# ducha-aiki/pydegensac

Measured on AMD Instinct MI355X. Metric: models/sec, findFundamentalMatrix @2000 corrs (LO-RANSAC + DEGENSAC, batched pairs), higher is better.
Workload: dtype f64

## Files before the change

pydegensac_amd/csrc/dg_f_lo.h:

```cpp
#ifndef DG_F_LO_H
#define DG_F_LO_H

__device__ __forceinline__ unsigned dg_hash_list(const int *list, int count, bool small_ids = false)
{
    if (count <= 0) return 0;
    const int lane = (int)(threadIdx.x & 63);
    unsigned hash = (unsigned)__builtin_amdgcn_readfirstlane(count * 4), tmp;
#define DG_HSTEP(v_) { unsigned v = (unsigned)(v_); \
        hash += v & 0xffffu; tmp = ((v >> 16) << 11) ^ hash; hash = (hash << 16) ^ tmp; hash += hash >> 11; }
#define DG_HSTEP16(v_) { unsigned v = (unsigned)(v_); \
        hash += v; hash = (hash << 16) ^ hash; hash += hash >> 11; }
    int k = 0;
    int cur = (lane < count) ? list[lane] : 0;
    int n1 = (64 + lane < count) ? list[64 + lane] : 0, n2 = (128 + lane < count) ? list[128 + lane] : 0, n3 = (192 + lane < count) ? list[192 + lane] : 0;
    for (; k + 64 <= count; k += 64) {
        const int n4 = (k + 256 + lane < count) ? list[k + 256 + lane] : 0;
        if (small_ids) {
#pragma unroll
            for (int i = 0; i < 64; i++) DG_HSTEP16(__builtin_amdgcn_readlane(cur, i))
        } else {
#pragma unroll
            for (int i = 0; i < 64; i++) DG_HSTEP(__builtin_amdgcn_readlane(cur, i))
        }
        cur = n1; n1 = n2; n2 = n3; n3 = n4;
// ... 64 lines not shown
        DG_LT(4);
        if (wv == 1) {
            unsigned hash = dg_hash_list(inliers, (int)Sc.I, n < 65536);
            if ((tid & 63) == 0) {
                int ret = dg_ht_contains(c.ht, hash, (int)Sc.I, iterID);
                if (ret == -1) dg_ht_insert(c.ht, hash, (int)Sc.I, iterID);
                S->itmp[0] = (ret != -1 && ret != iterID) ? 1 : 0;
            }
        } else if (wv == 0 && fit) {
            const int cnt = (int)r2.nL; int use = cnt, id;
            if (tid == 0) S->rng_save = S->rng;
            DG_WSYNC();
            if (8 < cnt) { dg_randsubset_wave(&S->rng, alt, cnt, 8, tid, &id); use = 8; }
            else id = tid < cnt ? alt[tid] : 0;
            if (tid < use) {
                dg_pt q = dg_ldpt<LDSPTS>(c.P, id);
                double *px = S->lsq.px + 4*tid; px[0] = q.x1; px[1] = q.y1; px[2] = q.x2; px[3] = q.y2;
                if (mk_ex == DG_K_FDS) S->lsq.part[0][tid] = dg_exFDs_w(fl, q.x1, q.y1, q.x2, q.y2);
                else { double w; dg_exFDsSym(fl, q.x1, q.y1, q.x2, q.y2, &w); S->lsq.part[0][tid] = w; }
            }
            DG_WSYNC();
            dg_u2f_small_w(&S->lsq, S->lsq.px, S->lsq.part[0], use, S->ftmp, tid);
        }
        __syncthreads();
        DG_LT(5);
        if (S->itmp[0]) {
            if (fit && tid == 0) S->rng = S->rng_save;
            __syncthreads();
            DG_TRACE(c, 13, 0, 0); return zero;
        }
        if (improve) {
            maxS = Sc; *kind0 = mk_ex;
            if (tid < 9) f[tid] = fl[tid];
        }
        DG_TRACE(c, 14, r2.nL, 0);
        for (int j = tid; j < (int)r2.nL; j += DG_T) inliers[j] = alt[j];
        if (tid < 9 && fit) fl[tid] = S->ftmp[tid];
        __syncthreads();
        DG_LT(6);
        if (!fit) return maxS;
        ths -= dth;
    }
    dg_pass_cfg c3 = dg_cfg0(n); c3.wantJ = 1; c3.thJ = th; c3.list = inliers; c3.thL = th;
    DG_LT(0);
    dg_pass_res r3 = dg_f_pass(c, fl, mk_full, c3); c.n_fds++;
    dg_dump_resid(c, rrow + 4, fl, mk_full);
    DG_LT(7);
    DG_TRACE(c, 12, r3.I, r3.J);
    if (maxS.J < r3.J) {
        maxS = zero; maxS.I = r3.I; maxS.J = r3.J; *kind0 = mk_full;
        __syncthreads();
        if (tid < 9) f[tid] = fl[tid];
        __syncthreads();
    }
    return maxS;
}

template <int LDSPTS>
__device__ __noinline__ dg_score dg_inFrani_serial(CTX &c, int ninl, double th, double *Fout, int *iterID,
                                               int mk_full, int mk_ex, int *kindBest)
{
    dg_f_shared *S = c.S; const int tid = c.tid;
    int *inliers = c.K->L[0], *intbuff = c.K->L[1], *intbuff_best = c.K->L[2];
    dg_score maxS = {0, 0, 0, 0};
    *kindBest = mk_full;
    if (ninl < 16) {
        if (c.rrun) { for (size_t j = tid; j < (size_t)(DG_RESIDS_M - 2) * c.n; j += DG_T) c.rrun[2 * (size_t)c.n + j] = 0.; __syncthreads(); }
        return maxS;
    }
    int ssiz = ninl / 2; if (ssiz > 14) ssiz = 14;
    const int wave = tid >> 6, lane = tid & 63;
    if (tid == 0) S->n_ahead = 0;
    for (int i = 0; i < DG_RAN_REP; i++) {
        DG_LT(0);
        __syncthreads();
        int taken = 0;
        if (S->n_ahead > 0) {
            if (tid < 64) {
                int hit = -1;
                for (int k = 0; k < S->n_ahead; k++) {
                    const int *a = (const int *)&S->rng, *b = (const int *)&S->ahead[k].before;
                    const bool same = lane < 31 ? a[lane] == b[lane] : (lane == 31 ? S->rng.f == S->ahead[k].before.f : (lane == 32
                        ? S->rng.b == S->ahead[k].before.b : true));
                    if (hit < 0 && __ballot(!same) == 0ull) hit = k;
                }
                if (hit >= 0) {
                    const dg_lo_ahead *h = &S->ahead[hit];
                    if (lane < 2 * ssiz && h->pos[lane] >= 0) inliers[h->pos[lane]] = h->val[lane];
                    if (lane < 9) S->f[lane] = h->F[lane];
                    DG_WSYNC();
                    if (lane == 0) S->rng = h->after;
                }
                if (lane == 0) S->itmp[29] = hit;
            }
            __syncthreads();
            taken = S->itmp[29] >= 0;
        }
        if (!taken) {
            if (tid < 64) { int id; dg_randsubset_wave(&S->rng, inliers, ninl, ssiz, tid, &id); dg_gather_wave(c, id, ssiz, S->lsq.px, tid); }
            __syncthreads();
            if (wave == 0) {
                dg_u2f_small_w(&S->lsq, S->lsq.px, 0, ssiz, S->f, tid);
            } else if (DG_AHEAD_ON && wave <= DG_LO_AHEAD && ssiz > 8 && i + 1 < DG_RAN_REP) {
                const int sub = wave == 1 ? 2 : wave == 2 ? 3 : wave == 3 ? 4 : wave == 4 ? 1 : 5;
                dg_lo_ahead *h = &S->ahead[wave - 1];
                dg_wave_ws *w = &S->ww[wave];
                if (lane == 0) { h->before = S->rng; for (int q = 0; q < 8 * sub; q++) dg_rand(&h->before); h->after = h->before; }
                DG_WSYNC();
                int id;
                dg_randsubset_wave_ahead(&h->after, inliers, ninl, ssiz, lane, &id, h->pos, h->val);
                dg_gather_wave(c, id, ssiz, w->px, lane);
                DG_WSYNC();
                dg_u2f_norm_w(w, w->px, (const double *)0, ssiz, h->F, lane);
            }
            if (tid == 0) S->n_ahead = (DG_AHEAD_ON && ssiz > 8 && i + 1 < DG_RAN_REP) ? DG_LO_AHEAD : 0;
        } else if (tid == 0) S->n_ahead = 0;
        DG_LT(8);
#ifdef DG_LO_PROF
        if (c.tid == 0) { if (taken) c.S->lt[10]++; else c.S->lt[11]++; }
#endif
        __syncthreads();
        int k0;
        ++*iterID;
        dg_dump_resid(c, 2 + 6 * i, S->f, mk_full);
        dg_score Sc = dg_iterF(c, intbuff, th, DG_TC * th, S->f, *iterID, mk_full, mk_ex, &k0, 2 + 6 * i + 1);
        if (maxS.J < Sc.J) {
            maxS = Sc; *kindBest = k0;
            __syncthreads();
            if (tid < 9) Fout[tid] = S->f[tid];
            for (int j = tid; j < (int)maxS.I; j += DG_T) intbuff_best[j] = intbuff[j];
            __syncthreads();
        }
    }
    __syncthreads();
    for (int j = tid; j < (int)maxS.I; j += DG_T) inliers[j] = intbuff_best[j];
    __syncthreads();
    return maxS;
}

template <int LDSPTS>
__device__ __forceinline__ dg_pass_res dg_f_wpass(const dg_pt *P, int n, int kind, const double *Fm , double thJ, int *la_, double thL, int *lb_,
    double thL2,
                                               double *tile, int lane)
{
    n = __builtin_amdgcn_readfirstlane(n); kind = __builtin_amdgcn_readfirstlane(kind);
    double F[9];
#pragma unroll
    for (int i = 0; i < 9; i++) F[i] = Fm[i];
    return dg_wpass_impl<LDSPTS>(P, n, [&](const dg_pt &q) { return dg_Ferr(kind, F, q); }, thJ, la_, thL, lb_, thL2, tile, lane);
}

#define DG_LO_ASSUMED_DRAWS 16
template <int LDSPTS>
__device__ __forceinline__ void dg_lo_rep_wave(CTX &c, dg_lo_log *lg, int ssiz, double th, int mk_full, int mk_ex, int lane, int wave)
{
    ssiz = __builtin_amdgcn_readfirstlane(ssiz); wave = __builtin_amdgcn_readfirstlane(wave);
    dg_f_shared *S = c.S; const int n = c.n, nm = c.K->n_max; const dg_pt *P = c.P;
    dg_wave_ws *w = &S->ww[wave];
    int *ib = c.K->wlist + (size_t)wave * nm;
    int *alt = (int *)(c.K->wstage + (size_t)wave * nm);
    double *jb = w->Z;
    double *f = w->F, *fl = w->H, *wts = w->cpx, *ftmp = w->cpx + 8;
    const bool small_ids = n < 65536;
#ifdef DG_LO_PROF
    long long tw_ = wall_clock64(); const long long tw0_ = tw_;
#define DG_RW(i) do { if (wave == 0 && lane == 0) { long long t_ = wall_clock64(); S->lt[i] += t_ - tw_; tw_ = t_; } } while (0)
#else
#define DG_RW(i) do {} while (0)
#endif
    auto stale = [&]() {
        int bad = 0;
        if (lane < wave) { const int d = __hip_atomic_load(&S->lo[lane].pub, __ATOMIC_RELAXED, __HIP_MEMORY_SCOPE_WORKGROUP);
            bad = d >= 0 && d != DG_LO_ASSUMED_DRAWS; }
        return __ballot(bad) != 0ull;
    };
    int drawn = 0;
    DG_WSYNC();
    dg_gather_wave(c, lane < ssiz ? lg->ids[lane] : 0, ssiz, w->px, lane);
    DG_WSYNC();
    dg_u2f_small_wave(w, w->px, (const double *)0, ssiz, f, lane);
    DG_RW(8);
    const dg_pass_res r0 = dg_f_wpass<LDSPTS>(P, n, mk_full, f, th, ib, th * DG_MWM, (int *)0, 0.0, jb, lane);
    DG_RW(9);
    unsigned mI = r0.I; double mJ = r0.J; int kind0 = mk_full;
    if (lane == 0) { lg->I0 = (int)r0.I; lg->drew0 = 0; lg->nit = 0; lg->has_fin = 0; }
    if (mI < 8) { if (lane == 0) { lg->I = 0; lg->J = 0; lg->kind0 = mk_full; __hip_atomic_store(&lg->pub, 0, __ATOMIC_RELAXED, __HIP_MEMORY_SCOPE_WORKGROUP);
        } DG_WSYNC(); return; }
    {
        const int cnt = (int)r0.nL; int id;
        if (8 < cnt) { dg_randsubset_wave(&lg->g, ib, cnt, 8, lane, &id); if (lane == 0) lg->drew0 = 8; drawn += 8; }
        else id = lane < cnt ? ib[lane] : 0;
        const int use = 8 < cnt ? 8 : cnt;
        DG_WSYNC();
        dg_gather_wave(c, id, use, w->px, lane);
        DG_WSYNC();
        dg_u2f_small_wave(w, w->px, (const double *)0, use, fl, lane);
    }
    DG_RW(10);
    double ths = DG_TC * th; const double dth = (ths - th) / DG_ILSQ_ITERS;
    int it = 0, ended = 0;
    for (; it < DG_ILSQ_ITERS; it++) {
        if (stale()) { if (lane == 0) lg->aborted = 1; DG_WSYNC(); return; }
        const dg_pass_res r1 = dg_f_wpass<LDSPTS>(P, n, mk_ex, fl, th, ib, th, alt, ths * DG_MWM, jb, lane);
        const int improve = __builtin_amdgcn_readfirstlane(mJ < r1.J);
        unsigned nL2 = r1.nL2;
        if (improve) { const dg_pass_res r2 = dg_f_wpass<LDSPTS>(P, n, kind0, f, 0.0, alt, ths * DG_MWM, (int *)0, 0.0, jb, lane); nL2 = r2.nL; }
        const int fit = __builtin_amdgcn_readfirstlane(nL2 >= 8);
        DG_WSYNC();
        DG_RW(9);
        const unsigned hash = dg_hash_list(ib, (int)r1.I, small_ids);
        if (lane == 0) { lg->it[it].hash = hash; lg->it[it].I = (int)r1.I; lg->it[it].drew = 0; lg->nit = it + 1; }
        { const bool known = dg_ht_known_wave(c.ht, hash, (int)r1.I, lane); DG_RW(11);
            if (known) { ended = 2; break; } }
        if (fit) {
            const int cnt = (int)nL2; int id;
            if (8 < cnt) {
                dg_randsubset_wave(&lg->g, alt, cnt, 8, lane, &id); if (lane == 0) lg->it[it].drew = 8; drawn += 8;
                if (drawn > DG_LO_ASSUMED_DRAWS && lane == 0) __hip_atomic_store(&lg->pub, drawn, __ATOMIC_RELAXED, __HIP_MEMORY_SCOPE_WORKGROUP);
            }
            else id = lane < cnt ? alt[lane] : 0;
            const int use = 8 < cnt ? 8 : cnt;
            DG_WSYNC();
            if (lane < use) {
                const dg_pt q = dg_ldpt<LDSPTS>(P, id);
                double *px = w->px + 4 * lane; px[0] = q.x1; px[1] = q.y1; px[2] = q.x2; px[3] = q.y2;
                if (mk_ex == DG_K_FDS) wts[lane] = dg_exFDs_w(fl, q.x1, q.y1, q.x2, q.y2);
                else { double ww_; dg_exFDsSym(fl, q.x1, q.y1, q.x2, q.y2, &ww_); wts[lane] = ww_; }
            }
            DG_WSYNC();
            dg_u2f_small_wave(w, w->px, wts, use, ftmp, lane);
        }
        if (improve) { mI = r1.I; mJ = r1.J; kind0 = mk_ex; DG_WSYNC(); if (lane < 9) f[lane] = fl[lane]; DG_WSYNC(); }
        for (int j = lane; j < (int)nL2; j += 64) ib[j] = alt[j];
        DG_WSYNC();
        if (lane < 9 && fit) fl[lane] = ftmp[lane];
        DG_WSYNC();
        DG_RW(10);
        if (!fit) { ended = 1; break; }
        ths -= dth;
    }
    if (!ended) {
        const dg_pass_res r3 = dg_f_wpass<LDSPTS>(P, n, mk_full, fl, th, ib, th, (int *)0, 0.0, jb, lane);
        if (lane == 0) lg->has_fin = 1;
        if (__builtin_amdgcn_readfirstlane(mJ < r3.J)) { mI = r3.I; mJ = r3.J; kind0 = mk_full; DG_WSYNC(); if (lane < 9) f[lane] = fl[lane]; DG_WSYNC(); }
    }
    DG_WSYNC();
    if (lane < 9) lg->f[lane] = f[lane];
#ifdef DG_LO_PROF
    DG_RW(9);
    if (wave == 0 && lane == 0) { S->lt[12] += wall_clock64() - tw0_; S->lt[13] += 100000; }
#endif
    if (lane == 0) { lg->I = (int)mI; lg->J = mJ; lg->kind0 = kind0; __hip_atomic_store(&lg->pub, drawn, __ATOMIC_RELAXED, __HIP_MEMORY_SCOPE_WORKGROUP); }
    DG_WSYNC();
}

template <int LDSPTS> __device__ __forceinline__ void dg_lo_round_coop(CTX &c, int nr, int ssiz, double th, int mk_full, int mk_ex);
__device__ __forceinline__ char *dg_coop_lojob(const dg_args &A, int slot);
__device__ __forceinline__ int *dg_coop_lo_list(const dg_args &A, int slot, int k);
template <int LDSPTS, bool COOP>
__device__ __noinline__ dg_score dg_inFrani_waves(CTX &c, int ninl, double th, double *Fout, int *iterID, int mk_full, int mk_ex, int *kindBest)
{
    dg_f_shared *S = c.S; const int tid = c.tid, lane = tid & 63, wave = tid >> 6;
    int *inliers = c.K->L[0], *intbuff_best = c.K->L[2];
    dg_score maxS = {0, 0, 0, 0};
    *kindBest = mk_full;
    if (ninl < 16) return maxS;
    int ssiz = ninl / 2; if (ssiz > 14) ssiz = 14;
    int next = 0;
    const int NRMAX = COOP ? DG_RAN_REP : ((c.A->lo_width > 0 && c.A->lo_width < DG_NW) ? c.A->lo_width : DG_NW);
    char *glog = (char *)0;
    if constexpr (COOP) glog = dg_coop_lojob(*c.A, c.coop_slot) + 128;
    auto LG = [&](int q) -> dg_lo_log * { if constexpr (COOP) return (dg_lo_log *)(glog + (size_t)DG_LOJOB_STRIDE * q); else return &S->lo[q]; };
    int assumed = COOP ? c.lo_assumed : DG_LO_ASSUMED_DRAWS;
#ifdef DG_LO_PROF
#define DG_LW(i) do { if (tid == 0) { long long t_ = wall_clock64(); S->lt[i] += t_ - S->ltq; S->ltq = t_; } } while (0)
#else
#define DG_LW(i) do {} while (0)
#endif
    while (next < DG_RAN_REP) {
        const int nr = DG_RAN_REP - next < NRMAX ? DG_RAN_REP - next : NRMAX;
        __syncthreads();
        DG_LW(7);
        if (__builtin_amdgcn_readfirstlane(wave) == 0) {
            if (lane == 0) S->lo_work = S->rng;
            DG_WSYNC();
            for (int q = 0; q < nr; q++) {
                dg_lo_log *g = LG(q);
                int id = 0;
                dg_randsubset_wave_ahead(&S->lo_work, inliers, ninl, ssiz, lane, &id, g->upos, g->uval);
                if (lane < ssiz) g->ids[lane] = id;
                if (lane < 2 * ssiz && g->upos[lane] >= 0) { const int old = inliers[g->upos[lane]]; inliers[g->upos[lane]] = g->uval[lane];
                    g->uval[lane] = old; }
                if (lane == 0) { g->g = S->lo_work; g->g0 = S->lo_work; g->pub = -1; g->aborted = 0; }
                DG_WSYNC();
                dg_rand_skip(&S->lo_work, assumed, lane);
            }
        }
        __syncthreads();
        DG_LW(0);
        if constexpr (COOP) dg_lo_round_coop<LDSPTS>(c, nr, ssiz, th, mk_full, mk_ex);
        else {
            const int wv = __builtin_amdgcn_readfirstlane(wave);
            if (wv < __builtin_amdgcn_readfirstlane(nr)) dg_lo_rep_wave<LDSPTS>(c, &S->lo[wv], ssiz, th, mk_full, mk_ex, lane, wv);
        }
        __syncthreads();
        DG_LW(1);
        if (tid == 0) {
            int v = 0;
            for (int q = 0; q < nr; q++) {
                dg_lo_log *g = LG(q);
                if (g->aborted) break;
                const int id = *iterID + next + q + 1;
                int draws = 0, cut = 0, n_ex = 0;
                if (g->I0 >= 8) {
                    draws = g->drew0;
                    for (int i = 0; i < g->nit; i++) {
                        n_ex++;
                        const int ret = dg_ht_contains(c.ht, g->it[i].hash, g->it[i].I, id);
                        if (ret == -1) dg_ht_insert(c.ht, g->it[i].hash, g->it[i].I, id);
                        if (ret != -1 && ret != id) { cut = 1; break; }
                        draws += g->it[i].drew;
                    }
                }
                g->cut = cut; g->draws = draws; g->n_ex = n_ex; g->n_fd = (!cut && g->has_fin) ? 2 : 1;
                v++;
                if (draws != assumed) break;
            }
            S->red.bi[0] = v;
        }
        __syncthreads();
        DG_LW(2);
        const int v = S->red.bi[0];
#ifdef DG_LO_PROF
        if (tid == 0) { S->lt[5] += 100000; S->lt[6] += 100000 * v; }
#endif
        for (int q = 0; q < v; q++) {
            const dg_lo_log *g = LG(q);
            c.n_exfds += g->n_ex; c.n_fds += g->n_fd;
            const int cut = g->cut;
            if (!cut && maxS.J < g->J) {
                maxS.I = (unsigned)g->I; maxS.J = g->J; maxS.Is = 0; maxS.Ilafs = 0; *kindBest = g->kind0;
                const int *ibq = COOP ? dg_coop_lo_list(*c.A, c.coop_slot, 2 * q) : c.K->wlist + (size_t)q * c.K->n_max;
                __syncthreads();
                if (tid < 9) Fout[tid] = g->f[tid];
                for (int j = tid; j < g->I; j += DG_T) intbuff_best[j] = ibq[j];
                __syncthreads();
            }
        }
        __syncthreads();
        DG_LW(3);
        if (__builtin_amdgcn_readfirstlane(wave) == 0) {
            for (int q = nr - 1; q >= v; q--) {
                if (lane < 2 * ssiz && LG(q)->upos[lane] >= 0) inliers[LG(q)->upos[lane]] = LG(q)->uval[lane];
                DG_WSYNC();
            }
            if (lane == 0) S->rng = LG(v - 1)->g0;
            DG_WSYNC();
            dg_rand_skip(&S->rng, LG(v - 1)->draws, lane);
        }
        next += v;
        if constexpr (COOP) {
            for (int q = 0; q < v; q++) { const int d = LG(q)->draws; if (d == c.lo_prev || c.lo_prev < 0) assumed = d; c.lo_prev = d; }
        }
#ifdef DG_LO_PROF
        __syncthreads();
#endif
        DG_LW(4);
    }
    if constexpr (COOP) c.lo_assumed = assumed;
    *iterID += DG_RAN_REP;
    __syncthreads();
    for (int j = tid; j < (int)maxS.I; j += DG_T) inliers[j] = intbuff_best[j];
    __syncthreads();
    return maxS;
}

template <int LDSPTS>
__device__ __forceinline__ dg_score dg_inFrani(CTX &c, int ninl, double th, double *Fout, int *iterID, int mk_full, int mk_ex, int *kindBest)
{
    if (c.rrun || c.A->innerh_serial || c.A->trace) return dg_inFrani_serial<LDSPTS>(c, ninl, th, Fout, iterID, mk_full, mk_ex, kindBest);
    if (c.cb) {
        if constexpr (LDSPTS == 0) return dg_inFrani_waves<LDSPTS, true>(c, ninl, th, Fout, iterID, mk_full, mk_ex, kindBest);
        else return dg_inFrani_serial<LDSPTS>(c, ninl, th, Fout, iterID, mk_full, mk_ex, kindBest);
    }
    return dg_inFrani_waves<LDSPTS, false>(c, ninl, th, Fout, iterID, mk_full, mk_ex, kindBest);
}

#endif
```

pydegensac_amd/csrc/dg_kernel_common.h:

```cpp
#ifndef DG_KERNEL_COMMON_H
#define DG_KERNEL_COMMON_H
#include "dg_geom.h"

#ifndef DG_CHUNK
#define DG_CHUNK   256
#endif
#ifdef MI_DEGENSAC_DEV
#define DG_CLK() wall_clock64()
#define DG_DEVT(x) x
#else
#define DG_CLK() 0ll
#define DG_DEVT(x) do {} while (0)
#endif
#ifndef DG_MINW
#define DG_MINW    2
#endif
#define DG_MCAP    96
#define DG_HT_CAP  4096
#define DG_MTAB_BYTES ((((size_t)3 * DG_CHUNK * 9 * sizeof(double)) + 255) & ~(size_t)255)
#define DG_PRE_BYTES  ((size_t)DG_CHUNK * 2 * sizeof(int))

#define DG_ITER_SAM 50
#define DG_RAN_REP 10
#define DG_ILSQ_ITERS 4
// ... 105 lines not shown
    int dev_knob;
    double *resids_out;
    int resid_runs;
    int lo_width;
    int *hist_out;
    int *screen_out;
    int *ticket;
    const int *order;
    int coop_k;
    int coop_pass_min;
    dg_coop_cb *coop;
    int park_sam;
    int n_res, n_ws;
    int dyn_bytes;
    int *park_ctl;
    long long *park_q;
    int park_cap;
    int park_long;
    int lo_serial;
    int pool_seq;
    int innerh_serial;
    int variant_threads, mode;
    int stream_on;
    int stream_early;
    int stream_min_sam, stream_min_left;
    int stream_depth;
    int stream_test;
    size_t stream_ent_bytes;
    dg_stream_cb *scb;
    char *ring;
    int *done_pairs;
    dg_hjob_cb *hjob;
    int fan_k;
    int fan_ws0;
    int *fan_flags;
    int *err_flag;
    int *trace;
    int trace_cap;
    int wait_ticks;
    long long *phase_out;
};

__device__ __forceinline__ bool dg_wait_count(const dg_args &A, int *cnt, int target, int code, int sleep_ticks)
{
    const long long t0 = wall_clock64(), limit = (long long)A.wait_ticks;
    for (;;) {
        const int v = __builtin_amdgcn_readfirstlane(__hip_atomic_load(cnt, __ATOMIC_RELAXED, __HIP_MEMORY_SCOPE_AGENT));
        if (v >= target && limit != 0) return true;
        if (wall_clock64() - t0 > limit || limit == 0) {
            if ((threadIdx.x & 63) == 0) __hip_atomic_store(A.err_flag, code, __ATOMIC_RELAXED, __HIP_MEMORY_SCOPE_AGENT);
            return false;
        }
        if (sleep_ticks >= 8) __builtin_amdgcn_s_sleep(8); else if (sleep_ticks >= 4) __builtin_amdgcn_s_sleep(4); else __builtin_amdgcn_s_sleep(2);
    }
}

static __constant__ unsigned dg_rng_C[8][32];
static __constant__ unsigned dg_rng_Ct[32][8];
static __constant__ unsigned dg_rng_G[32];
static __constant__ unsigned dg_rng_T[31][32];

__device__ __forceinline__ unsigned dg_mulmod31(unsigned a, unsigned b)
{
    unsigned long long x = (unsigned long long)a * b;
    x = (x & 0x7fffffffull) + (x >> 31);
    x = (x & 0x7fffffffull) + (x >> 31);
    if (x >= 0x7fffffffull) x -= 0x7fffffffull;
    return (unsigned)x;
}
__device__ __forceinline__ unsigned dg_lcg_first(int r0)
{
    if (r0 >= 0) return dg_mulmod31((unsigned)r0, 16807u);
    long long hi = r0 / 127773, lo = r0 % 127773;
    long long word = 16807 * lo - 2836 * hi;
    if (word < 0) word += 2147483647;
    return (unsigned)word;
}
__device__ __forceinline__ void dg_rng_outputs(unsigned seed, unsigned *o)
{
    if (seed == 0) seed = 1;
    unsigned r1 = dg_lcg_first((int)seed);
    unsigned acc[8];
#pragma unroll
    for (int k = 0; k < 8; k++) acc[k] = dg_rng_Ct[0][k] * seed;
    (void)r1;
    for (int j = 1; j < 31; j++) {
        unsigned rj = dg_mulmod31(seed < 0x7fffffffu ? seed : r1, seed < 0x7fffffffu ? dg_rng_G[j] : dg_rng_G[j - 1]);
#pragma unroll
        for (int k = 0; k < 8; k++) acc[k] += dg_rng_Ct[j][k] * rj;
    }
#pragma unroll
    for (int k = 0; k < 8; k++) o[k] = acc[k] >> 1;
}
__device__ __forceinline__ unsigned dg_rng_next_seed_wave(unsigned seed, int lane, int kout = 7)
{
    if (seed == 0) seed = 1;
    unsigned r1 = dg_lcg_first((int)seed);
    unsigned rj = (lane == 0) ? seed : ((lane < 31) ? dg_mulmod31(r1, dg_rng_G[(lane - 1) & 31]) : 0u);
    unsigned term = (lane < 31) ? dg_rng_C[kout][lane & 31] * rj : 0u;
    return dg_wave_sum_u(term) >> 1;
}

__device__ __forceinline__ void dg_srand_wave(dg_rng *g, unsigned seed, int lane)
{
    if (seed == 0) seed = 1;
    const unsigned r1 = dg_lcg_first((int)seed);
    const unsigned rj = lane == 0 ? seed : (lane < 31 ? dg_mulmod31(r1, dg_rng_G[(lane - 1) & 31]) : 0u);
    const int p = lane < 31 ? lane : 0;
    unsigned acc = 0;
#pragma unroll
    for (int j = 0; j < 31; j++) acc += dg_rng_T[j][p] * (unsigned)__builtin_amdgcn_readlane((int)rj, j);
    DG_WSYNC();
    if (lane < 31) g->r[lane] = (int32_t)acc;
    if (lane == 0) { g->f = 3; g->b = 0; }
    DG_WSYNC();
}
__device__ __forceinline__ int dg_rand_block(dg_rng *g, int n, int lane)
{
    const int f = g->f, b = g->b;
    int idx = f + (lane < 31 ? lane : 30); if (idx >= 31) idx -= 31;
    const unsigned s = (unsigned)g->r[idx];
    unsigned x = lane < 31 ? s : 0u, t;
    t = (unsigned)__shfl_up((int)x, 3, 64);  if (lane >= 3)  x += t;
    t = (unsigned)__shfl_up((int)x, 6, 64);  if (lane >= 6)  x += t;
    t = (unsigned)__shfl_up((int)x, 12, 64); if (lane >= 12) x += t;
    t = (unsigned)__shfl_up((int)x, 24, 64); if (lane >= 24) x += t;
    const unsigned o = x + (unsigned)__shfl((int)s, 28 + lane % 3, 64);
    DG_WSYNC();
    if (lane < n) g->r[idx] = (int32_t)o;
    if (lane == 0) { int nf = f + n, nb = b + n; g->f = nf >= 31 ? nf - 31 : nf; g->b = nb >= 31 ? nb - 31 : nb; }
    DG_WSYNC();
    return (int)(o >> 1);
}
__device__ __forceinline__ void dg_rand_skip(dg_rng *g, int n, int lane)
{
    n = __builtin_amdgcn_readfirstlane(n);
    while (n > 0) { const int m = n > 31 ? 31 : n; (void)dg_rand_block(g, m, lane); n -= m; }
}

struct dg_ht { int *heads; int *ent; int *count; };
__device__ __forceinline__ void dg_ht_init(dg_ht &h, int tid)
{
    if (tid < 64) h.heads[tid] = -1;
    if (tid == 0) *h.count = 0;
}
__device__ __forceinline__ int dg_ht_contains(const dg_ht &h, unsigned hash, int length, int iterID)
{
    int e = h.heads[hash % 64];
    while (e >= 0) { if ((unsigned)h.ent[4*e] == hash && h.ent[4*e+1] == length && h.ent[4*e+2] == iterID) return iterID; e = h.ent[4*e+3]; }
    e = h.heads[hash % 64];
    while (e >= 0) { if ((unsigned)h.ent[4*e] == hash && h.ent[4*e+1] == length) return h.ent[4*e+2]; e = h.ent[4*e+3]; }
    return -1;
}
__device__ __forceinline__ bool dg_ht_known_wave(const dg_ht &h, unsigned hash, int length, int lane)
{
    typedef __attribute__((address_space(1))) int dg_gint;
    const dg_gint *ent = (const dg_gint *)h.ent;
    const int cnt = __builtin_amdgcn_readfirstlane(*(const dg_gint *)h.count);
    bool hit = false;
    for (int e = lane; e < cnt; e += 64) hit = hit || ((unsigned)ent[4*e] == hash && ent[4*e+1] == length);
    return __ballot(hit) != 0ull;
}
__device__ __forceinline__ void dg_ht_insert(dg_ht &h, unsigned hash, int length, int iterID)
{
    int e = *h.count;
    if (e >= DG_HT_CAP) return;
    h.ent[4*e] = (int)hash; h.ent[4*e+1] = length; h.ent[4*e+2] = iterID; h.ent[4*e+3] = h.heads[hash % 64];
    h.heads[hash % 64] = e; *h.count = e + 1;
}

__device__ __forceinline__ int dg_randsubset(dg_rng *g, int *pool, int max_sz, int siz)
{
    for (int i = 0; i < siz; i++) {
        int s = dg_rand(g) % (max_sz - i);
        int j = max_sz - i - 1;
        int q = pool[s]; pool[s] = pool[j]; pool[j] = q;
    }
    return max_sz - siz;
}


__device__ __forceinline__ int dg_randsubset_wave(dg_rng *g, int *pool, int max_sz, int siz, int lane, int *id)
{
    int myS = 0;
    if (siz <= 31) { const int raw_ = dg_rand_block(g, siz, lane); if (lane < siz) myS = raw_ % (max_sz - lane); }
    else for (int i = 0; i < siz; i++) {
        int s = 0;
        if (lane == 0) s = dg_rand(g) % (max_sz - i);
        s = __builtin_amdgcn_readfirstlane(s);
        if (lane == i) myS = s;
    }
    const bool used = lane < 2 * siz;
    const int drawn = __shfl(myS, lane >= siz ? lane - siz : 0, 64);
    const int pos = lane < siz ? max_sz - 1 - lane : (used ? drawn : -1);
    int val = used ? pool[pos] : 0;
    for (int i = 0; i < siz; i++) {
        const int s_i = __builtin_amdgcn_readlane(myS, i), t_i = max_sz - 1 - i;
        const unsigned long long mA = __ballot(used && pos == s_i), mB = __ballot(used && pos == t_i);
        const int la = __ffsll((long long)mA) - 1, lb = __ffsll((long long)mB) - 1;
        const int va = __builtin_amdgcn_readlane(val, la), vb = __builtin_amdgcn_readlane(val, lb);
        if (lane == la) val = vb;
        if (lane == lb) val = va;
    }
    bool canon = used;
    for (int j = 0; j < 2 * siz; j++) { const int pj = __builtin_amdgcn_readlane(pos, j); if (j < lane && pj == pos) canon = false; }
    if (canon) pool[pos] = val;
    *id = __shfl(val, lane < siz ? siz - 1 - lane : 0, 64);
    return max_sz - siz;
}

__device__ __forceinline__ void dg_randsubset_wave_ahead(dg_rng *g, const int *pool, int max_sz, int siz, int lane, int *id, int *pos_out, int *val_out)
{
    int myS = 0;
    if (siz <= 31) { const int raw_ = dg_rand_block(g, siz, lane); if (lane < siz) myS = raw_ % (max_sz - lane); }
    else for (int i = 0; i < siz; i++) {
        int s = 0;
        if (lane == 0) s = dg_rand(g) % (max_sz - i);
        s = __builtin_amdgcn_readfirstlane(s);
        if (lane == i) myS = s;
    }
    const bool used = lane < 2 * siz;
    const int drawn = __shfl(myS, lane >= siz ? lane - siz : 0, 64);
    const int pos = lane < siz ? max_sz - 1 - lane : (used ? drawn : -1);
    int val = used ? pool[pos] : 0;
    for (int i = 0; i < siz; i++) {
        const int s_i = __builtin_amdgcn_readlane(myS, i), t_i = max_sz - 1 - i;
        const unsigned long long mA = __ballot(used && pos == s_i), mB = __ballot(used && pos == t_i);
        const int la = __ffsll((long long)mA) - 1, lb = __ffsll((long long)mB) - 1;
        const int va = __builtin_amdgcn_readlane(val, la), vb = __builtin_amdgcn_readlane(val, lb);
        if (lane == la) val = vb;
        if (lane == lb) val = va;
    }
    bool canon = used;
    for (int j = 0; j < 2 * siz; j++) { const int pj = __builtin_amdgcn_readlane(pos, j); if (j < lane && pj == pos) canon = false; }
    if (used) { pos_out[lane] = canon ? pos : -1; val_out[lane] = val; }
    *id = __shfl(val, lane < siz ? siz - 1 - lane : 0, 64);
}

#endif
```

pydegensac_amd/csrc/dg_kernel_f.h:

```cpp
#ifndef DG_KERNEL_F_H
#define DG_KERNEL_F_H
#include <stddef.h>
#include "dg_lsq.h"

struct dg_score { unsigned I; double J; unsigned Is; unsigned Ilafs; };

#define DG_WPAD ((2 * DG_CHUNK * 7 * 4 > DG_NW * (int)sizeof(dg_wave_ws)) ? (2 * DG_CHUNK * 7 * 4 - DG_NW * (int)sizeof(dg_wave_ws) + 7) / 8 : 1)
struct dg_f_drv {
    dg_score maxS, maxSs;
    int no_sam, max_sam, iter_cnt, degen_cnt, iterID, Ihmax; unsigned non_degen;
    int best_sample; long long t_best, t_start;
    long long t_parked;
    int flast_k, has_last;
    int finKind, accepted, perm[4], p4, e4kind, track, done;
    unsigned seed; int cur, chunk_s[3], chunk_base;
    int n_fds, n_exfds, n_hds, n_aux;
};

#ifndef DG_LO_AHEAD_MAX
#define DG_LO_AHEAD_MAX 5
#endif
#define DG_LO_AHEAD (DG_NW - 1 < DG_LO_AHEAD_MAX ? DG_NW - 1 : DG_LO_AHEAD_MAX)
struct dg_lo_ahead { dg_rng before, after; int pos[32], val[32]; double F[9]; };

#define DG_LSQ_LTAB(S) (sizeof((S)->ww) + sizeof((S)->wpad) >= 640 * sizeof(double) ? (double *)(S)->ww : (double *)0)

struct dg_f_cshared {
    int *L[10];
    unsigned char *Fl[5];
    double *gmodels;
    dg_pt *stage;
    unsigned *res_I; double *res_J;
    int (*rf)[5];
    int *wlist; dg_pt *wstage;
    char *hrep;
    int n_max;
};

struct dg_ih_log { dg_rng g; double h[9]; double itJ; int ids[12]; int passes, draws;
                   int pub, aborted; };

struct dg_lo_it { unsigned hash; int I; int drew; };
struct dg_lo_log {
    dg_rng g, g0;
    int upos[28], uval[28];
    int ids[14];
    int I0, drew0, nit, has_fin;
    dg_lo_it it[DG_ILSQ_ITERS];
    double f[9], J; int I, kind0;
    int cut, draws, n_ex, n_fd;
    int pub, aborted;
};
#define DG_LOJOB_STRIDE 768
#define DG_LOJOB_BYTES (128 + DG_RAN_REP * DG_LOJOB_STRIDE)
static_assert(sizeof(dg_lo_log) <= DG_LOJOB_STRIDE, "dg_lo_log does not fit its slot");
struct dg_lo_job { int n, ssiz, mk_full, mk_ex; double th; };

struct dg_f_shared {
    dg_red red;
    dg_lsq_scratch lsq;
    dg_rng rng, rng_save;
    unsigned seeds3[3][DG_CHUNK];
    int      draws3[3][DG_CHUNK][8];
    unsigned long long alm3[3][DG_CHUNK / 64];
    dg_wave_ws ww[DG_NW];
    double   wpad[DG_WPAD];
    double   csH[5][9]; int csRes[5];
    union {
        struct {
            double   fhF[16][9], fhF2[16][9], fhTh[16];
            int      fhIds[16][10], fhCnt[16], fhCnt2[16], fhRaw[160];
        };
        dg_lo_ahead ahead[DG_LO_AHEAD];
        struct { dg_ih_log ih[DG_NW]; dg_rng ih_start, ih_work; };
        struct { dg_lo_log lo[DG_NW]; dg_rng lo_start, lo_work; };
    };
    int n_ahead;
    int n_lafrej;
    unsigned scnt[4];
    long long ph[8], dbg[8], tq;
#ifdef DG_LO_PROF
    long long lt[16], ltq;
#endif
    unsigned short moff[DG_T + 1];
    unsigned char  nv[DG_CHUNK];
    unsigned char  ridx[DG_CHUNK][4];
    unsigned short mslot[3 * DG_CHUNK];
    unsigned wave_cnt[DG_NW];
    double   f[9], F[9], FBest[9], H[9], Hx[9], fLO[9], ftmp[9];
    double   bufF[4][9]; int bufKind[4];
    double   u7[7][4];
    double   ext[4], extw[DG_NW][4];
    int      samidxBest[7];
    int      itmp[32];
    unsigned char nsolv[DG_CHUNK];
    double   flast[9]; int lastIds[8];
    double   dtmp[32];
    dg_f_drv park;
    dg_f_cshared K;
};

struct dg_stream_ev { double model[9]; double J; unsigned I; short k; unsigned char r, pad; unsigned char ridx[4]; };
#define DG_STREAM_EV_MAX 40
struct dg_stream_ent {
    int cn, Mtot, n_ev, overflow; double tau_used, pad1;
    unsigned seeds[DG_CHUNK]; int draws[DG_CHUNK][8];
    unsigned char nv[DG_CHUNK];
    dg_stream_ev ev[DG_STREAM_EV_MAX];
};

template <int LDSPTS>
struct dg_f_ctx {
    dg_f_shared *S;
    const __attribute__((address_space(3))) dg_f_cshared *K;
    const dg_pt *P;
    int *pool;
    int n, tid;
    const dg_args *A;
    long long off;
    dg_ht ht;
    unsigned *seeds; int (*draws)[8];
    int n_fds, n_exfds, n_hds, n_aux;
    double *rrun;
    dg_coop_cb *cb; int *coop_gen; int coop_slot;
    double *hlt;
    int hjob_gen;
    int lo_assumed, lo_prev;

    __device__ __forceinline__ dg_pt pt(int i) const { return P[i]; }
    __device__ __forceinline__ dg_pt laf_pt(int i, int which) const {
        const double *a = A->pts1 + (size_t)(off + i) * 6, *b = A->pts2 + (size_t)(off + i) * 6;
        dg_pt p;
        if (which == 1) { p.x1 = a[0] + a[3]; p.y1 = a[1] + a[5]; p.x2 = b[0] + b[3]; p.y2 = b[1] + b[5]; }
        else            { p.x1 = a[0] + a[2]; p.y1 = a[1] + a[4]; p.x2 = b[0] + b[2]; p.y2 = b[1] + b[4]; }
        return p;
    }
};

#define DG_JBUF_LDS_BYTES (offsetof(dg_f_shared, wpad) + sizeof(((dg_f_shared *)0)->wpad) - offsetof(dg_f_shared, ww))
static_assert(offsetof(dg_f_shared, wpad) == offsetof(dg_f_shared, ww) + sizeof(((dg_f_shared *)0)->ww), "ww and wpad must be contiguous");
static_assert(DG_JBUF_LDS_BYTES >= 2 * DG_CHUNK * 7 * sizeof(int), "pool-stage scratch does not fit");

__device__ __forceinline__ void dg_fill_views(dg_f_cshared *K, char *ws, const dg_ws_layout &wl)
{
    for (int i = 0; i < 10; i++) K->L[i] = (int *)(ws + wl.off_lists) + (size_t)i * wl.n_max;
    for (int i = 0; i < 5; i++) K->Fl[i] = (unsigned char *)(ws + wl.off_flags) + (size_t)i * wl.n_max;
    K->gmodels = (double *)(ws + wl.off_models);
    K->stage = (dg_pt *)(ws + wl.off_stage);
    K->res_J = (double *)(ws + wl.off_res); K->res_I = (unsigned *)(K->res_J + 3 * DG_CHUNK); K->rf = (int (*)[5])(K->res_I + 3 * DG_CHUNK);
    K->hrep = wl.hrep ? ws + wl.off_hrep : (char *)0;
    K->n_max = wl.n_max; K->wlist = (int *)(ws + wl.off_wave); K->wstage = (dg_pt *)(ws + wl.off_wave + (size_t)DG_NW * wl.n_max * sizeof(int));
}

#define CTX dg_f_ctx<LDSPTS>
#define DG_RESIDS_M 62

template <int LDSPTS>
__device__ __forceinline__ void dg_dump_resid(CTX &c, int row, const double *M, int kind)
{
    if (!c.rrun) return;
    double m[9], Hinv[9], H1[9];
#pragma unroll
    for (int i = 0; i < 9; i++) { m[i] = M[i]; Hinv[i] = 0; H1[i] = 0; }
    if (kind > 10) dg_hsym_prepare(m, Hinv, H1);
    double *out = c.rrun + (size_t)row * c.n;
    for (int j = c.tid; j < c.n; j += DG_T) {
        const dg_pt q = dg_ldpt<LDSPTS>(c.P, j);
        out[j] = kind < 10 ? dg_Ferr(kind, m, q) : dg_Herr(kind - 10, m, Hinv, H1, q);
    }
}
template <int LDSPTS>
__device__ __forceinline__ void dg_resid_begin(CTX &c, int run )
{
    c.rrun = 0;
    if (!c.A->resids_out || run >= c.A->resid_runs) return;
    c.rrun = c.A->resids_out + ((size_t)c.off * c.A->resid_runs + (size_t)run * c.n) * DG_RESIDS_M;
    const double nan_ = __longlong_as_double(0x7ff8000000000000ll);
    for (size_t j = c.tid; j < (size_t)DG_RESIDS_M * c.n; j += DG_T) c.rrun[j] = nan_;
}

#define DG_TRACE(c, tag, I, J) do { if ((c).A->trace && (c).tid == 0) { int *t_ = (c).A->trace; int k_ = t_[0]; \
    if (k_ < (c).A->trace_cap) { long long jb_ = __double_as_longlong((double)(J)); t_[1+4*k_] = (tag); t_[2+4*k_] = (int)(I); \
    t_[3+4*k_] = (int)(jb_ & 0xffffffffll); t_[4+4*k_] = (int)(jb_ >> 32); t_[0] = k_ + 1; } } } while (0)

template <int LDSPTS>
__device__ __noinline__ dg_pass_res dg_coop_pass(CTX &c, const double *Fm , int kind, const dg_pass_cfg &cfg);

template <int LDSPTS>
__device__ __forceinline__ dg_pass_res dg_f_pass(CTX &c, const double *Fm , int kind, dg_pass_cfg cfg)
{
    if (LDSPTS == 0 && c.cb && !cfg.src && !cfg.flags && !cfg.wantC && cfg.n >= c.A->coop_pass_min) return dg_coop_pass<LDSPTS>(c, Fm, kind, cfg);
    double F[9];
#pragma unroll
    for (int i = 0; i < 9; i++) F[i] = Fm[i];
    const dg_pt *P = c.P;
    cfg.jbuf = (double *)c.K->stage; cfg.jl = (double *)c.S->ww; cfg.jl_cap = (int)(DG_JBUF_LDS_BYTES / sizeof(double));
    return dg_pass(&c.S->red, cfg, [&](int pid, int) { return dg_Ferr(kind, F, dg_ldpt<LDSPTS>(P, pid)); }, c.tid);
}
template <int LDSPTS>
__device__ __forceinline__ dg_pass_res dg_h_pass(CTX &c, const double *Hm , dg_pass_cfg cfg)
{
    double H[9];
#pragma unroll
    for (int i = 0; i < 9; i++) H[i] = Hm[i];
    const dg_pt *P = c.P;
    cfg.jbuf = (double *)c.K->stage; cfg.jl = (double *)c.S->ww; cfg.jl_cap = (int)(DG_JBUF_LDS_BYTES / sizeof(double));
    return dg_pass(&c.S->red, cfg, [&](int pid, int) { dg_pt p = dg_ldpt<LDSPTS>(P, pid); return dg_HDs(H, p.x1, p.y1, p.x2, p.y2); }, c.tid);
}
__device__ __forceinline__ dg_pass_cfg dg_cfg0(int n)
{
    dg_pass_cfg c; c.n = n; c.src = 0; c.p0 = 0; c.wantJ = 0; c.thJ = 0; c.jbuf = 0; c.jl = 0; c.jl_cap = 0; c.wantC = 0; c.thC = 0; c.list = 0; c.thL = 0;
        c.listStrict = 0; c.list2 = 0; c.thL2 = 0; c.flags = 0; c.thF = 0;
    return c;
}

template <int LDSPTS>
__device__ __forceinline__ void dg_gather(CTX &c, const int *ids, int len, double *px)
{
    for (int i = 0; i < len; i++) { dg_pt p = dg_ldpt<LDSPTS>(c.P, ids[i]); px[4*i] = p.x1; px[4*i+1] = p.y1; px[4*i+2] = p.x2; px[4*i+3] = p.y2; }
}

template <int LDSPTS>
__device__ __forceinline__ void dg_gather_wave(CTX &c, int id, int len, double *px, int lane)
{
    if (lane < len) { dg_pt p = dg_ldpt<LDSPTS>(c.P, id); px[4*lane] = p.x1; px[4*lane+1] = p.y1; px[4*lane+2] = p.x2; px[4*lane+3] = p.y2; }
}

template <int LDSPTS>
// ... 796 lines not shown
```

Baseline: 97.28 million.

## Replace round-synchronous LO repetitions with a lock-based sliding window scheduler

Per-wave local-optimization repetitions no longer run in lockstep rounds separated by workgroup barriers. Waves now take a shared lock, commit finished repetitions in order (hash-table inserts, RNG replay, best-model update) and claim new speculative repetitions in a sliding window. A repetition is rolled back and restarted through epoch counters when its assumed draw count turns out wrong. This is meant to remove idle time at the barriers when repetitions differ in cost. In exchange it adds spin-waiting, atomics, an abort timeout and more complex correctness conditions.

```diff
diff --git a/pydegensac_amd/csrc/dg_f_lo.h b/pydegensac_amd/csrc/dg_f_lo.h
--- a/pydegensac_amd/csrc/dg_f_lo.h
+++ b/pydegensac_amd/csrc/dg_f_lo.h
@@ -240,13 +240,15 @@
 
 #define DG_LO_ASSUMED_DRAWS 16
 template <int LDSPTS>
-__device__ __forceinline__ void dg_lo_rep_wave(CTX &c, dg_lo_log *lg, int ssiz, double th, int mk_full, int mk_ex, int lane, int wave)
-{
-    ssiz = __builtin_amdgcn_readfirstlane(ssiz); wave = __builtin_amdgcn_readfirstlane(wave);
+__device__ __forceinline__ void dg_lo_rep_wave(CTX &c, dg_lo_log *lg, int slot, int q, int ep, int W, int ssiz, double th, int mk_full, int mk_ex,
+                                               int lane, int wave)
+{
+    ssiz = __builtin_amdgcn_readfirstlane(ssiz); wave = __builtin_amdgcn_readfirstlane(wave); slot = __builtin_amdgcn_readfirstlane(slot);
+    q = __builtin_amdgcn_readfirstlane(q); ep = __builtin_amdgcn_readfirstlane(ep); W = __builtin_amdgcn_readfirstlane(W);
     dg_f_shared *S = c.S; const int n = c.n, nm = c.K->n_max; const dg_pt *P = c.P;
     dg_wave_ws *w = &S->ww[wave];
-    int *ib = c.K->wlist + (size_t)wave * nm;
-    int *alt = (int *)(c.K->wstage + (size_t)wave * nm);
+    int *ib = c.K->wlist + (size_t)slot * nm;
+    int *alt = (int *)(c.K->wstage + (size_t)slot * nm);
     double *jb = w->Z;
     double *f = w->F, *fl = w->H, *wts = w->cpx, *ftmp = w->cpx + 8;
     const bool small_ids = n < 65536;
@@ -258,8 +260,12 @@
 #endif
     auto stale = [&]() {
         int bad = 0;
-        if (lane < wave) { const int d = __hip_atomic_load(&S->lo[lane].pub, __ATOMIC_RELAXED, __HIP_MEMORY_SCOPE_WORKGROUP);
-            bad = d >= 0 && d != DG_LO_ASSUMED_DRAWS; }
+        if (lane < W) { const dg_lo_log *o = &S->lo[lane];
+            const int r = __hip_atomic_load(&o->rep, __ATOMIC_RELAXED, __HIP_MEMORY_SCOPE_WORKGROUP);
+            const int e = __hip_atomic_load(&o->ep, __ATOMIC_RELAXED, __HIP_MEMORY_SCOPE_WORKGROUP);
+            const int d = __hip_atomic_load(&o->pub, __ATOMIC_RELAXED, __HIP_MEMORY_SCOPE_WORKGROUP);
+            bad = r >= 0 && r < q && e == ep && d >= 0 && d != DG_LO_ASSUMED_DRAWS; }
+        if (lane == 0) bad |= __hip_atomic_load(&S->lo_win.ep, __ATOMIC_RELAXED, __HIP_MEMORY_SCOPE_WORKGROUP) != ep;
         return __ballot(bad) != 0ull;
     };
     int drawn = 0;
@@ -268,6 +274,7 @@
     DG_WSYNC();
     dg_u2f_small_wave(w, w->px, (const double *)0, ssiz, f, lane);
     DG_RW(8);
+    if (stale()) { if (lane == 0) lg->aborted = 1; DG_WSYNC(); return; }
     const dg_pass_res r0 = dg_f_wpass<LDSPTS>(P, n, mk_full, f, th, ib, th * DG_MWM, (int *)0, 0.0, jb, lane);
     DG_RW(9);
     unsigned mI = r0.I; double mJ = r0.J; int kind0 = mk_full;
@@ -298,7 +305,7 @@
         DG_RW(9);
         const unsigned hash = dg_hash_list(ib, (int)r1.I, small_ids);
         if (lane == 0) { lg->it[it].hash = hash; lg->it[it].I = (int)r1.I; lg->it[it].drew = 0; lg->nit = it + 1; }
-        { const bool known = dg_ht_known_wave(c.ht, hash, (int)r1.I, lane); DG_RW(11);
+        { const bool known = dg_ht_known_wave<true>(c.ht, hash, (int)r1.I, lane); DG_RW(11);
             if (known) { ended = 2; break; } }
         if (fit) {
             const int cnt = (int)nL2; int id;
@@ -340,6 +347,194 @@
 #endif
     if (lane == 0) { lg->I = (int)mI; lg->J = mJ; lg->kind0 = kind0; __hip_atomic_store(&lg->pub, drawn, __ATOMIC_RELAXED, __HIP_MEMORY_SCOPE_WORKGROUP); }
     DG_WSYNC();
+}
+
+#define DG_LDS_LD(x) __hip_atomic_load(&(x), __ATOMIC_RELAXED, __HIP_MEMORY_SCOPE_WORKGROUP)
+#define DG_LDS_ST(x, v) __hip_atomic_store(&(x), (v), __ATOMIC_RELAXED, __HIP_MEMORY_SCOPE_WORKGROUP)
+template <int LDSPTS>
+__device__ __forceinline__ void dg_lo_window(CTX &c, int ninl, int ssiz, double th, double *Fout, int iter0, int mk_full, int mk_ex)
+{
+    dg_f_shared *S = c.S; const int tid = c.tid, lane = tid & 63;
+    const int wave = __builtin_amdgcn_readfirstlane(tid >> 6);
+    int *inliers = c.K->L[0], *intbuff_best = c.K->L[2];
+    dg_lo_win *Wn = &S->lo_win;
+    const int W = __builtin_amdgcn_readfirstlane((c.A->lo_width > 0 && c.A->lo_width < DG_NW) ? c.A->lo_width : DG_NW);
+    const long long lim = c.A->wait_ticks > 0 ? (long long)c.A->wait_ticks : 400000000ll;
+    __syncthreads();
+    if (tid == 0) {
+        Wn->lock = 0; Wn->h = 0; Wn->p = 0; Wn->ep = 0; Wn->abort = 0; Wn->nex = 0; Wn->nfd = 0; Wn->kind = mk_full; Wn->I = 0; Wn->J = 0.0;
+        S->lo_work = S->rng; Wn->htc = *c.ht.count;
+    }
+    if (tid < DG_RAN_REP + 2) Wn->slot_of[tid] = -1;
+    if (tid < DG_NW) { S->lo[tid].rep = -1; S->lo[tid].ep = -1; S->lo[tid].done = 0; S->lo[tid].busy = 0; S->lo[tid].pub = -1; }
+    __syncthreads();
+#ifdef DG_LO_PROF
+#define DG_LWW(i, t0_) do { if (lane == 0) S->lt[i] += wall_clock64() - (t0_); } while (0)
+#else
+#define DG_LWW(i, t0_) do {} while (0)
+#endif
+    auto free_slot = [&](int h, int e) {
+        int fr = 0;
+        if (lane < W) { const dg_lo_log *o = &S->lo[lane];
+            const int r = DG_LDS_LD(o->rep), oe = DG_LDS_LD(o->ep);
+            fr = !DG_LDS_LD(o->busy) && (r < h || oe != e); }
+        const unsigned long long m = __ballot(fr);
+        return m ? (int)__builtin_ctzll(m) : -1;
+    };
+    auto brk = [&](int hb) {
+        const int p = __builtin_amdgcn_readfirstlane(Wn->p);
+        for (int q = p - 1; q >= hb; q--) {
+            const dg_lo_log *o = &S->lo[__builtin_amdgcn_readfirstlane(Wn->slot_of[q])];
+            if (lane < 2 * ssiz && o->upos[lane] >= 0) inliers[o->upos[lane]] = o->uval[lane];
+            DG_WSYNC();
+        }
+        if (lane == 0) { S->lo_work = S->rng; Wn->p = hb; DG_LDS_ST(Wn->ep, Wn->ep + 1); }
+        DG_WSYNC();
+#ifdef DG_LO_PROF
+        if (lane == 0) S->lt[5] += 100000;
+#endif
+    };
+    long long tw = wall_clock64();
+    for (;;) {
+        const int h = __builtin_amdgcn_readfirstlane(DG_LDS_LD(Wn->h));
+        if (h >= DG_RAN_REP || __builtin_amdgcn_readfirstlane(DG_LDS_LD(Wn->abort))) break;
+        int act;
+        {
+            const int p = __builtin_amdgcn_readfirstlane(DG_LDS_LD(Wn->p)), e = __builtin_amdgcn_readfirstlane(DG_LDS_LD(Wn->ep));
+            const int sh = __builtin_amdgcn_readfirstlane(DG_LDS_LD(Wn->slot_of[h]));
+            act = sh >= 0 ? __builtin_amdgcn_readfirstlane((int)(DG_LDS_LD(S->lo[sh].done) && DG_LDS_LD(S->lo[sh].rep) == h
+                                                                 && DG_LDS_LD(S->lo[sh].ep) == e)) : 0;
+            if (!act && p < DG_RAN_REP && p < h + W) act = free_slot(h, e) >= 0;
+        }
+        int got = 0;
+        if (act && lane == 0) { int e = 0;
+            got = __hip_atomic_compare_exchange_strong(&Wn->lock, &e, 1, __ATOMIC_ACQUIRE, __ATOMIC_RELAXED, __HIP_MEMORY_SCOPE_WORKGROUP) ? 1 : 0; }
+        got = __builtin_amdgcn_readfirstlane(got);
+        if (!got) {
+            if (wall_clock64() - tw > lim) {
+                if (lane == 0) { __hip_atomic_store(c.A->err_flag, 32, __ATOMIC_RELAXED, __HIP_MEMORY_SCOPE_AGENT); DG_LDS_ST(Wn->abort, 1); }
+                break;
+            }
+            __builtin_amdgcn_s_sleep(1);
+            continue;
+        }
+        __builtin_amdgcn_fence(__ATOMIC_ACQUIRE, "workgroup");
+#ifdef DG_LO_PROF
+        const long long tl0_ = wall_clock64();
+#endif
+        for (;;) {
+            const int h = __builtin_amdgcn_readfirstlane(Wn->h);
+            if (h >= DG_RAN_REP) break;
+            const int slot = __builtin_amdgcn_readfirstlane(Wn->slot_of[h]);
+            if (slot < 0) break;
+            dg_lo_log *g = &S->lo[slot];
+            const int ready = __builtin_amdgcn_readfirstlane((int)(DG_LDS_LD(g->done) && DG_LDS_LD(g->rep) == h && DG_LDS_LD(g->ep) == Wn->ep));
+            if (!ready) break;
+            __builtin_amdgcn_fence(__ATOMIC_ACQUIRE, "workgroup");
+            if (__builtin_amdgcn_readfirstlane(g->aborted)) { brk(h); break; }
+            const int id = iter0 + h + 1;
+            int draws = 0, cut = 0, n_ex = 0;
+            if (__builtin_amdgcn_readfirstlane(g->I0) >= 8) {
+                draws = __builtin_amdgcn_readfirstlane(g->drew0);
+                const int nit = __builtin_amdgcn_readfirstlane(g->nit);
+                const int cnt0 = __builtin_amdgcn_readfirstlane(Wn->htc);
+                int cntw = cnt0, own_in = 0;
+                int ins_e[DG_ILSQ_ITERS], ins_b[DG_ILSQ_ITERS];
+                typedef __attribute__((address_space(1))) int dg_gint;
+                const dg_gint *ent = (const dg_gint *)c.ht.ent;
+                for (int i = 0; i < nit; i++) {
+                    n_ex++;
+                    const unsigned hs = (unsigned)__builtin_amdgcn_readfirstlane((int)g->it[i].hash);
+                    const int len = __builtin_amdgcn_readfirstlane(g->it[i].I);
+                    int own = 0;
+                    for (int j = 0; j < i; j++)
+                        if (((own_in >> j) & 1) && (unsigned)g->it[j].hash == hs && g->it[j].I == len) own = 1;
+                    own = __builtin_amdgcn_readfirstlane(own);
+                    const int hd = lane == 0 ? ((const dg_gint *)c.ht.heads)[hs % 64] : 0;
+                    int best = -1, bid = -1;
+                    for (int e = lane; e < cnt0; e += 64)
+                        if ((unsigned)ent[4*e] == hs && ent[4*e+1] == len) { best = e; bid = ent[4*e+2]; }
+#pragma unroll
+                    for (int o = 32; o >= 1; o >>= 1) {
+                        const int tb = __shfl_xor(best, o, 64), ti = __shfl_xor(bid, o, 64);
+                        if (tb > best) { best = tb; bid = ti; }
+                    }
+                    const int ret = own ? id : (__builtin_amdgcn_readfirstlane(best) < 0 ? -1 : __builtin_amdgcn_readfirstlane(bid));
+                    if (ret == -1) {
+                        if (cntw < DG_HT_CAP) {
+                            const int b = (int)(hs % 64);
+                            int nxt = __builtin_amdgcn_readfirstlane(hd);
+                            for (int j = 0; j < i; j++) if (((own_in >> (8 + j)) & 1) && ins_b[j] == b) nxt = ins_e[j];
+                            if (lane == 0) { int *en = c.ht.ent + 4 * cntw; en[0] = (int)hs; en[1] = len; en[2] = id; en[3] = nxt; c.ht.heads[b] = cntw; }
+                            ins_e[i] = cntw; ins_b[i] = b; cntw++;
+                            own_in |= (1 << i) | (1 << (8 + i));
+                        }
+                    } else if (ret == id) own_in |= 1 << i;
+                    if (ret != -1 && ret != id) { cut = 1; break; }
+                    draws += __builtin_amdgcn_readfirstlane(g->it[i].drew);
+                }
+                if (cntw != cnt0) {
+                    if (lane == 0) { __hip_atomic_store(c.ht.count, cntw, __ATOMIC_RELEASE, __HIP_MEMORY_SCOPE_WORKGROUP); Wn->htc = cntw; }
+                    DG_WSYNC();
+                }
+            }
+            const int n_fd = (!cut && __builtin_amdgcn_readfirstlane(g->has_fin)) ? 2 : 1;
+            if (lane == 0) { g->cut = cut; g->draws = draws; g->n_ex = n_ex; g->n_fd = n_fd; Wn->nex += n_ex; Wn->nfd += n_fd; }
+            if (__builtin_amdgcn_readfirstlane((int)(!cut && Wn->J < g->J))) {
+                const int I = __builtin_amdgcn_readfirstlane(g->I);
+                const int *ibq = c.K->wlist + (size_t)slot * c.K->n_max;
+                if (lane == 0) { Wn->I = (unsigned)I; Wn->J = g->J; Wn->kind = g->kind0; }
+                if (lane < 9) Fout[lane] = g->f[lane];
+                for (int j = lane; j < I; j += 64) intbuff_best[j] = ibq[j];
+            }
+            if (lane == 0) S->rng = g->g0;
+            DG_WSYNC();
+            dg_rand_skip(&S->rng, draws, lane);
+            if (lane == 0) DG_LDS_ST(Wn->h, h + 1);
+            DG_WSYNC();
+#ifdef DG_LO_PROF
+            if (lane == 0) S->lt[6] += 100000;
+#endif
+            if (draws != DG_LO_ASSUMED_DRAWS) { if (h + 1 < DG_RAN_REP) brk(h + 1); break; }
+        }
+        DG_LWW(2, tl0_);
+        int my = -1, myq = 0, myep = 0;
+        {
+#ifdef DG_LO_PROF
+            const long long tp0_ = wall_clock64();
+#endif
+            const int h = __builtin_amdgcn_readfirstlane(Wn->h), p = __builtin_amdgcn_readfirstlane(Wn->p);
+            const int ep = __builtin_amdgcn_readfirstlane(Wn->ep);
+            const int slot = (p < DG_RAN_REP && p < h + W) ? free_slot(h, ep) : -1;
+            if (slot >= 0) {
+                dg_lo_log *g = &S->lo[slot];
+                int id = 0;
+                dg_randsubset_wave_ahead(&S->lo_work, inliers, ninl, ssiz, lane, &id, g->upos, g->uval);
+                if (lane < ssiz) g->ids[lane] = id;
+                if (lane < 2 * ssiz && g->upos[lane] >= 0) { const int old = inliers[g->upos[lane]]; inliers[g->upos[lane]] = g->uval[lane];
+                    g->uval[lane] = old; }
+                if (lane == 0) {
+                    g->g = S->lo_work; g->g0 = S->lo_work; g->aborted = 0; g->done = 0; Wn->slot_of[p] = slot;
+                    DG_LDS_ST(g->pub, -1); DG_LDS_ST(g->rep, p); DG_LDS_ST(g->ep, ep); DG_LDS_ST(g->busy, 1); DG_LDS_ST(Wn->p, p + 1);
+                }
+                DG_WSYNC();
+                dg_rand_skip(&S->lo_work, DG_LO_ASSUMED_DRAWS, lane);
+                my = slot; myq = p; myep = ep;
+                DG_LWW(0, tp0_);
+            }
+        }
+        __builtin_amdgcn_fence(__ATOMIC_RELEASE, "workgroup");
+        if (lane == 0) __hip_atomic_store(&Wn->lock, 0, __ATOMIC_RELAXED, __HIP_MEMORY_SCOPE_WORKGROUP);
+        my = __builtin_amdgcn_readfirstlane(my);
+        if (my >= 0) {
+            dg_lo_rep_wave<LDSPTS>(c, &S->lo[my], my, myq, myep, W, ssiz, th, mk_full, mk_ex, lane, wave);
+            __builtin_amdgcn_fence(__ATOMIC_RELEASE, "workgroup");
+            if (lane == 0) { DG_LDS_ST(S->lo[my].done, 1); DG_LDS_ST(S->lo[my].busy, 0); }
+        }
+        tw = wall_clock64();
+    }
+#undef DG_LWW
+    __syncthreads();
 }
 
 template <int LDSPTS> __device__ __forceinline__ void dg_lo_round_coop(CTX &c, int nr, int ssiz, double th, int mk_full, int mk_ex);
@@ -362,9 +557,16 @@
     int assumed = COOP ? c.lo_assumed : DG_LO_ASSUMED_DRAWS;
 #ifdef DG_LO_PROF
 #define DG_LW(i) do { if (tid == 0) { long long t_ = wall_clock64(); S->lt[i] += t_ - S->ltq; S->ltq = t_; } } while (0)
+    const long long tlo0_ = wall_clock64();
 #else
 #define DG_LW(i) do {} while (0)
 #endif
+    if constexpr (!COOP) {
+        dg_lo_window<LDSPTS>(c, ninl, ssiz, th, Fout, *iterID, mk_full, mk_ex);
+        maxS.I = S->lo_win.I; maxS.J = S->lo_win.J; *kindBest = S->lo_win.kind;
+        c.n_exfds += S->lo_win.nex; c.n_fds += S->lo_win.nfd;
+        next = DG_RAN_REP;
+    }
     while (next < DG_RAN_REP) {
         const int nr = DG_RAN_REP - next < NRMAX ? DG_RAN_REP - next : NRMAX;
         __syncthreads();
@@ -387,10 +589,6 @@
         __syncthreads();
         DG_LW(0);
         if constexpr (COOP) dg_lo_round_coop<LDSPTS>(c, nr, ssiz, th, mk_full, mk_ex);
-        else {
-            const int wv = __builtin_amdgcn_readfirstlane(wave);
-            if (wv < __builtin_amdgcn_readfirstlane(nr)) dg_lo_rep_wave<LDSPTS>(c, &S->lo[wv], ssiz, th, mk_full, mk_ex, lane, wv);
-        }
         __syncthreads();
         DG_LW(1);
         if (tid == 0) {
@@ -460,6 +658,9 @@
     __syncthreads();
     for (int j = tid; j < (int)maxS.I; j += DG_T) inliers[j] = intbuff_best[j];
     __syncthreads();
+#ifdef DG_LO_PROF
+    if (tid == 0) { S->lt[14] += wall_clock64() - tlo0_; S->lt[15] += 100000; }
+#endif
     return maxS;
 }
 
diff --git a/pydegensac_amd/csrc/dg_kernel_common.h b/pydegensac_amd/csrc/dg_kernel_common.h
--- a/pydegensac_amd/csrc/dg_kernel_common.h
+++ b/pydegensac_amd/csrc/dg_kernel_common.h
@@ -281,11 +281,13 @@
     while (e >= 0) { if ((unsigned)h.ent[4*e] == hash && h.ent[4*e+1] == length) return h.ent[4*e+2]; e = h.ent[4*e+3]; }
     return -1;
 }
+template <bool CONCURRENT = false>
 __device__ __forceinline__ bool dg_ht_known_wave(const dg_ht &h, unsigned hash, int length, int lane)
 {
     typedef __attribute__((address_space(1))) int dg_gint;
     const dg_gint *ent = (const dg_gint *)h.ent;
-    const int cnt = __builtin_amdgcn_readfirstlane(*(const dg_gint *)h.count);
+    const int cnt = __builtin_amdgcn_readfirstlane(CONCURRENT ? __hip_atomic_load(h.count, __ATOMIC_ACQUIRE, __HIP_MEMORY_SCOPE_WORKGROUP)
+                                                              : *(const dg_gint *)h.count);
     bool hit = false;
     for (int e = lane; e < cnt; e += 64) hit = hit || ((unsigned)ent[4*e] == hash && ent[4*e+1] == length);
     return __ballot(hit) != 0ull;
diff --git a/pydegensac_amd/csrc/dg_kernel_f.h b/pydegensac_amd/csrc/dg_kernel_f.h
--- a/pydegensac_amd/csrc/dg_kernel_f.h
+++ b/pydegensac_amd/csrc/dg_kernel_f.h
@@ -50,7 +50,9 @@
     double f[9], J; int I, kind0;
     int cut, draws, n_ex, n_fd;
     int pub, aborted;
+    int rep, ep, done, busy;
 };
+struct dg_lo_win { int lock, h, p, ep, abort, nex, nfd, kind; unsigned I; int htc; double J; int slot_of[DG_RAN_REP + 2]; };
 #define DG_LOJOB_STRIDE 768
 #define DG_LOJOB_BYTES (128 + DG_RAN_REP * DG_LOJOB_STRIDE)
 static_assert(sizeof(dg_lo_log) <= DG_LOJOB_STRIDE, "dg_lo_log does not fit its slot");
@@ -73,7 +75,7 @@
         };
         dg_lo_ahead ahead[DG_LO_AHEAD];
         struct { dg_ih_log ih[DG_NW]; dg_rng ih_start, ih_work; };
-        struct { dg_lo_log lo[DG_NW]; dg_rng lo_start, lo_work; };
+        struct { dg_lo_log lo[DG_NW]; dg_rng lo_start, lo_work; dg_lo_win lo_win; };
     };
     int n_ahead;
     int n_lafrej;
```

Measured after the change: 98.03 million, median of 6. About the same (+0.8%).
